# acoustic-warfare/beamforming-lk

Measured on AMD Instinct MI355X. Metric: heatmap frames/sec, higher is better.
Workload: dtype f32

## Files before the change

beamforming-lk_amd/_build.py:

```python
from __future__ import annotations

import os
import shutil
import subprocess
from pathlib import Path

PKG_DIR = Path(__file__).resolve().parent
REPO = PKG_DIR.parent
CSRC = PKG_DIR / "csrc"
LIB_PATH = PKG_DIR / "libawpu_hip.so"

SOURCES = [CSRC / "das_kernels.hip", CSRC / "das_fast.hip", CSRC / "track_kernels.hip", CSRC / "block_kernels.hip", CSRC / "watch_kernels.hip",
           CSRC / "awpu_hip.cpp", CSRC / "awpu_group.cpp", CSRC / "awpu_sweep.cpp", CSRC / "awpu_runs.cpp", CSRC / "geometry_host.cpp"]
GENERATOR = REPO / "tools" / "gen_trip_asm.py"
TRIP_INC = CSRC / "das_fast_trip.inc"
HEADERS = [CSRC / "awpu_handle.h", CSRC / "das_kernels.h", CSRC / "block_kernels.h", CSRC / "watch_kernels.h", GENERATOR, REPO / "include" / "awpu_hip.h", REPO / "include" / "awpu_hip_track.h",
           REPO / "include" / "awpu_hip_blocks.h", REPO / "include" / "awpu_hip_listen.h", REPO / "include" / "awpu_hip_watch.h"]


def hipcc_path() -> str:
    for cand in (os.environ.get("HIPCC"), shutil.which("hipcc"), "/opt/rocm/bin/hipcc"):
        if cand and Path(cand).exists():
            return cand
    raise RuntimeError("hipcc not found: libawpu_hip.so cannot be built (there is no CPU fallback)")


def stale() -> bool:
    if not LIB_PATH.exists():
        return True
    built = LIB_PATH.stat().st_mtime
    return any(p.stat().st_mtime > built for p in SOURCES + HEADERS)
# ... 62 lines not shown
```

beamforming-lk_amd/csrc/awpu_handle.h:

```cpp
#pragma once

#include "awpu_hip.h"
#include "awpu_hip_track.h"

#include <hip/hip_runtime.h>

#include <algorithm>
#include <string>
#include <utility>
#include <vector>

#include "das_kernels.h"

namespace awpu::host {

void note_error(const std::string &text);

struct CtxScope {
    awpu_hip *saved;
    explicit CtxScope(awpu_hip *h);
    ~CtxScope();
};
#define AWPU_CTX(h) awpu::host::CtxScope ctx_scope_(h)

// ... 195 lines not shown
    bool have_table = false, have_mics = false, prepared = false;

    Dev<awpu::LutEntry> d_lut;
    struct FastLut {
        awpu::FastPlan plan;
        Dev<awpu::FastEntry> d;
        size_t entries = 0;
    };
    std::vector<FastLut> fast_luts;
    Dev<awpu::FastEntry> d_exact_pair_lut;
    size_t exact_pair_lut_entries = 0, fir_plane_lut_entries = 0;
    awpu::FastPlan exact_plan{};
    awpu::host::QuadTable quad_tables[awpu::host::kQuadLayouts];
    Dev<unsigned> d_nd_queue;
    Dev<int2> d_nd_items;
    long long nd_items_key = -1;
    int n_cus = 0;
    bool exact_nd_ok = false;
    bool exact_ndh_ok = false, exact_ndhs_ok = false, fast_ndp_ok = false;
    bool identity_mics = false;
    bool exact_pairs_ok = false;
    float *sums_out = nullptr;
    Dev<uint32_t> d_fir_plane_lut;
    awpu::FastPlan fir_plane_plan{};
    bool fir_planes_ok = false;
    std::vector<float> fir;
    bool quadh_fits = false;
    bool quadhs_fits = false;
    bool quad_ok = false;
    double quad_cost = 0.0;
// ... 156 lines not shown
```

beamforming-lk_amd/csrc/awpu_sweep.cpp:

```cpp
#include "awpu_handle.h"

#include <algorithm>
#include <array>
#include <cstdio>
#include <cstdlib>
#include <cstring>
#include <map>
#include <vector>

#include "das_kernels.h"

using namespace awpu::host;

namespace {

int diag_begin(awpu_hip *h, size_t words, bool zero, hipStream_t s, unsigned long long **out) {
    if (const int rc = h->d_diag.ensure(words); rc != AWPU_OK) return rc;
    if (zero) AWPU_HIP_TRY(hipMemsetAsync(h->d_diag, 0, words * sizeof(unsigned long long), s));
    *out = h->d_diag;
    return AWPU_OK;
}

int diag_end(awpu_hip *h, int rc, size_t n_waves, int wg_waves, const char *tag, hipStream_t s) {
    if (rc != AWPU_OK || n_waves == 0) return rc;
    AWPU_HIP_TRY(hipStreamSynchronize(s));
// ... 76 lines not shown
    return AWPU_OK;
}
#endif

int ensure_pack(awpu_hip *h, size_t need) { return ensure_seen_by_live_graphs(h, h->d_pack, need); }

}

namespace awpu::host {

void free_tables(awpu_hip *h) {
    h->d_lut.release();
    h->fast_luts.clear();
    h->d_exact_pair_lut.release();
    for (QuadTable &q : h->quad_tables) q.d.release();
    h->d_fir_plane_lut.release();
}

int prepare(awpu_hip *h) {
    const auto &c = h->cfg;
    const int U = h->usable();
    const int P = c.pixel_count;
    int lo = c.hist, hi = -1;
    for (int p = 0; p < P; p++) {
        const int32_t *row = &h->off[(size_t) p * c.lut_stride];
        for (int s = 0; s < U; s++) {
            const int o = row[h->index[s]];
            lo = std::min(lo, o);
            hi = std::max(hi, o);
        }
// ... 41 lines not shown
                for (int q = 0; q < 2; q++) rr[2 * s + q] = h->index[s] * 2048 + lo + q;
            if (const int rc = h->d_row_off_ring.grow(rr.size()); rc != AWPU_OK) return rc;
            AWPU_HIP_TRY(hipMemcpy(h->d_row_off_ring, rr.data(), rr.size() * sizeof(int32_t), hipMemcpyHostToDevice));
        }
        if (h->compact_hist) {
            for (int s = 0; s < U; s++)
                for (int q = 0; q < 2; q++) ro[2 * s + q] = h->index[s] * h->compact_hist + q;
            for (size_t i = 2 * (size_t) U; i < ro.size(); i++) ro[i] = h->index[0] * h->compact_hist;
            if (const int rc = h->d_row_off_compact.grow(ro.size()); rc != AWPU_OK) return rc;
            AWPU_HIP_TRY(hipMemcpy(h->d_row_off_compact, ro.data(), ro.size() * sizeof(int32_t), hipMemcpyHostToDevice));
        }
    }

    h->exact_pairs_ok = c.math == AWPU_MATH_F32_EXACT && c.interp == AWPU_INTERP_LERP && awpu::pair_plan(h->window, U, &h->exact_plan);
    h->quad_tables[kQuadExact].plan = h->exact_plan;
    h->exact_nd_ok = h->exact_pairs_ok && awpu::exact_nd_plan(h->window, U, &h->quad_tables[kQuadExactNd].plan);
    h->exact_ndh_ok = h->exact_pairs_ok && awpu::exact_ndh_plan(h->window, U, false, &h->quad_tables[kQuadExactNdh].plan);
    h->fast_ndp_ok = c.math == AWPU_MATH_F32_FAST && c.interp == AWPU_INTERP_LERP && awpu::exact_ndh_plan(h->window, U, false, &h->quad_tables[kQuadExactNdh].plan);
    h->exact_ndhs_ok = h->exact_pairs_ok && awpu::exact_ndh_plan(h->window, U, true, &h->quad_tables[kQuadExactNdhStationary].plan);
    h->fir_planes_ok = c.math == AWPU_MATH_F32_FAST && c.interp == AWPU_INTERP_FIR8 && awpu::fir8_plane_plan(h->window, U, &h->fir_plane_plan);
    if (c.math != AWPU_MATH_F32_FAST || c.interp == AWPU_INTERP_FIR8) {
        int chunk = 0;
        if (awpu::das_exact_lds_bytes(h->window, U, &chunk) == 0)
            return invalid("delay window does not fit the LDS budget");
        std::vector<awpu::LutEntry> packed((size_t) P * U);
        for (int p = 0; p < P; p++) {
            const int32_t *orow = &h->off[(size_t) p * c.lut_stride];
            const float *frow = &h->frac[(size_t) p * c.lut_stride];
            awpu::LutEntry *dst = &packed[(size_t) p * U];
            for (int s = 0; s < U; s++) {
                const int id = h->index[s];
// ... 127 lines not shown
    }
    if (const int rc = lut.d.grow(n); rc != AWPU_OK) return rc;
    AWPU_HIP_TRY(hipMemcpy(lut.d, packed.data(), n * sizeof(awpu::FastEntry), hipMemcpyHostToDevice));
    lut.entries = n;
    h->fast_luts.reserve(8);
    h->fast_luts.push_back(std::move(lut));
    *out = &h->fast_luts.back();
    return AWPU_OK;
}

int build_quad_lut(awpu_hip *h, QuadLayout layout) {
    QuadTable &table = h->quad_tables[layout];
    if (table.d) return AWPU_OK;
    const auto &c = h->cfg;
    const awpu::FastPlan &plan = table.plan;
    const bool halves_nd = layout == kQuadExactNdh || layout == kQuadExactNdhStationary;
    const bool raw = layout == kQuadExact || layout == kQuadExactNd || halves_nd;
    const float centre = raw ? 0.0f : 0.5f;
    const int elem = layout == kQuadExactNd || halves_nd ? 16 : 8;
    const int U = h->usable(), cols = c.grid_columns, rows = c.pixel_count / cols;
    const int groups = plan.usable_pad / 4;
    const int cols_pad = halves_nd ? (cols + 31) / 32 * 32 : (cols + 15) / 16 * 16, rows4 = layout == kQuadExactNd ? ((rows + 3) / 4 + 1) / 2 * 2 : (rows + 3) / 4;
    const size_t n = (size_t) rows4 * cols_pad * groups * 16 + 2 * awpu::kQuadTablePrefetch;
    std::vector<awpu::QuadEntry> packed(n, awpu::QuadEntry{0.0f, 0u});
    for (int r4 = 0; r4 < rows4; r4++)
        for (int col = 0; col < cols_pad; col++) {
            awpu::QuadEntry *dst = &packed[((size_t) r4 * cols_pad + col) * groups * 16];
            for (int q = 0; q < 4; q++) {
                const int row = 4 * r4 + q;
                const bool inside = row < rows && col < cols;
                const size_t p = (size_t) std::min(row, rows - 1) * cols + std::min(col, cols - 1);
                const int32_t *orow = &h->off[p * c.lut_stride];
                const float *frow = &h->frac[p * c.lut_stride];
                for (int s = 0; s < plan.usable_pad; s++) {
                    awpu::QuadEntry &e = dst[((s >> 2) * 4 + q) * 4 + (s & 3)];
                    const int j = s % plan.chunk;
                    if (s < U) {
                        const int id = h->index[s];
                        const int off_rel = orow[id] - h->wstart;
                        e.f = inside ? frow[id] - centre : 0.0f;
                        e.addr = (uint32_t) (j * plan.row_bytes + off_rel * elem);
                    } else {
                        e.f = 0.0f;
                        e.addr = (uint32_t) (j * plan.row_bytes);
                    }
                }
            }
        }
    if (const int rc = table.d.grow(n); rc != AWPU_OK) return rc;
    AWPU_HIP_TRY(hipMemcpy(table.d, packed.data(), n * sizeof(awpu::QuadEntry), hipMemcpyHostToDevice));
    table.entries = n;
    return AWPU_OK;
}

// ... 165 lines not shown

int launch_exact_nd(awpu_hip *h, const float *d_frames, int batch, float *d_power, hipStream_t s, int hist_eff, int wstart_eff, int nq,
                    const float *prepacked = nullptr, size_t prepacked_floats = 0) {
    int rc = build_quad_lut(h, kQuadExactNd);
    if (rc != AWPU_OK) return rc;
    const QuadTable &table = h->quad_tables[kQuadExactNd];
    const awpu::FastPlan &pp = table.plan;
    if (!prepacked)
        if (const int prc = ensure_pack(h, pair_pack_floats(std::max(h->cfg.max_batch, batch), pp.usable_pad, pp.wr, 4)); prc != AWPU_OK) return prc;
    awpu::ExactNdArgs a{};
    fill_shared(a, h, pp, batch, d_power);
    a.packed = prepacked ? prepacked : h->d_pack;
    a.lut = table.d;
    a.sums = h->sums_out;
    a.wq = pp.wr;
    a.cols = h->cfg.grid_columns;
    a.rows = h->cfg.pixel_count / a.cols;
    a.nq = nq;
    a.tiles = awpu::nd_tiles(a.rows, a.cols, nq);
    a.n_pairs = (batch + 1) / 2;
    a.pair_group = xcd_pair_group((size_t) pp.usable_pad * pp.row_bytes, a.n_pairs);
    {
        const size_t items = (size_t) a.n_pairs * a.tiles;
        const long long key = ((long long) a.n_pairs << 24) | ((long long) a.pair_group << 8) | nq;
        if (!h->d_nd_items.holds(items)) {
            retire_live_graphs(h);
            AWPU_HIP_TRY(hipStreamSynchronize(s));
            if (rc = h->d_nd_items.grow(items); rc != AWPU_OK) return rc;
            h->nd_items_key = -1;
        }
        a.items = h->d_nd_items;
        a.build_items = h->nd_items_key != key;
        h->nd_items_key = key;
    }
    if (rc = arm_item_queues(h, a.n_pairs * a.tiles, &a.queue, &a.wgs, &a.tail); rc != AWPU_OK) return rc;
#ifdef AWPU_TUNING_BUILD
    if (const char *v = std::getenv("AWPU_ND_TAIL")) {
        const int per = (a.n_pairs * a.tiles + 7) / 8;
        a.tail = std::max(1, std::atoi(v) >= 100 ? per : per * std::atoi(v) / 100);
    }
#endif
    if (h->timing) AWPU_HIP_TRY(hipEventRecord(h->ev_begin, s));
    if (!prepacked)
        AWPU_HIP_TRY(awpu::launch_pack_nd(d_frames, h->cfg.n_streams, hist_eff, wstart_eff, h->d_index, h->usable(), pp.usable_pad, h->d_gain,
                                          pp.wr, batch, h->d_pack, s));
#ifdef AWPU_TUNING_BUILD
    const size_t n_wgs = std::min<size_t>((size_t) a.n_pairs * a.tiles, (size_t) a.wgs);
    if (env().debug & 16)
        if (const int drc = diag_begin(h, n_wgs * 8, true, s, &a.debug_out); drc != AWPU_OK) return drc;
#endif
    AWPU_HIP_TRY(awpu::launch_das_exact_nd(a, {table.entries, prepacked ? prepacked_floats : h->d_pack.cap}, s));
    rc = finish_launch(h, batch, s, AWPU_KERNEL_EXACT_ND);
#ifdef AWPU_TUNING_BUILD
    if (rc == AWPU_OK && (env().debug & 16)) return dump_nd_timeline(h, n_wgs, s);
#endif
    return rc;
}

bool takes_exact_nd(awpu_hip *h, int batch, int *nq) {
    if (!h->exact_pairs_ok || !h->exact_nd_ok || h->cfg.grid_columns < 1) return false;
// ... 425 lines not shown

bool takes_packed_pairs(awpu_hip *h, int batch, awpu::FastPlan *plan) {
    if (batch < 2 || h->cfg.interp != AWPU_INTERP_LERP || h->usable() % 4 != 0 || !h->gain.empty()) return false;
    if (h->cfg.math == AWPU_MATH_F32_EXACT) {
        int nq = 1;
        if (!takes_exact_nd(h, batch, &nq)) return false;
        *plan = h->quad_tables[kQuadExactNd].plan;
        return true;
    }
    if (h->cfg.math != AWPU_MATH_F32_FAST || env().pairs == 0) return false;
    if (!awpu::pair_plan(h->window, h->usable(), plan)) return false;
    return (fast_batch_takes_quads(h, batch) && quad_plan_is(h, *plan)) || fast_batch_takes_pairs(h, batch);
}

size_t packed_floats_of(const awpu_hip *h, const awpu::FastPlan &plan, int batch) {
    return (size_t) ((batch + 1) / 2) * h->usable() * (size_t) (plan.row_bytes / 4);
}

int pack_for_sweep(awpu_hip *h, const awpu::FastPlan &plan, const float *d_frames, int batch, float *d_packed, hipStream_t s) {
    if (h->cfg.math == AWPU_MATH_F32_EXACT)
        AWPU_HIP_TRY(awpu::launch_pack_nd(d_frames, h->cfg.n_streams, h->cfg.hist, h->wstart, h->d_index, h->usable(), h->usable(), nullptr, plan.wr,
                                          batch, d_packed, s));
    else
        AWPU_HIP_TRY(awpu::launch_pack_pairs(d_frames, h->cfg.n_streams, h->cfg.hist, h->wstart, h->d_index, h->usable(), h->usable(), nullptr,
                                             plan.wr, batch, d_packed, true, s));
    return AWPU_OK;
}

int sweep_packed(awpu_hip *h, const awpu::FastPlan &plan, const float *d_packed, size_t packed_floats, int batch, float *d_power,
                 hipStream_t s) {
    if (h->cfg.math == AWPU_MATH_F32_EXACT) {
        int nq = 1;
        if (!takes_exact_nd(h, batch, &nq)) return fail(AWPU_ERR_STATE, "packed frames: this batch is not swept by the {next, d} kernel");
        return launch_exact_nd(h, nullptr, batch, d_power, s, h->cfg.hist, h->wstart, nq, d_packed, packed_floats);
    }
    if (fast_batch_takes_quads(h, batch) && quad_plan_is(h, plan))
        return launch_quads(h, nullptr, batch, d_power, s, h->cfg.hist, h->wstart, d_packed, packed_floats);
// ... 24 lines not shown
```

beamforming-lk_amd/csrc/das_fast.hip:

```cpp
#include "das_kernels.h"

#include <algorithm>
#include <atomic>

namespace awpu {

typedef float f2 __attribute__((ext_vector_type(2)));
typedef float f4 __attribute__((ext_vector_type(4)));
typedef float f4u __attribute__((ext_vector_type(4), aligned(4)));
typedef float f8 __attribute__((ext_vector_type(8)));

#define AWPU_AS4 __attribute__((address_space(4)))

typedef int i16 __attribute__((ext_vector_type(16)));

struct EntryGroup {
    i16 v;
    __device__ __forceinline__ float f(int k) const { return __int_as_float(v[4 * k + 0]); }
    __device__ __forceinline__ unsigned addr(int k) const { return (unsigned) v[4 * k + 1]; }
    __device__ __forceinline__ float g(int k) const { return __int_as_float(v[4 * k + 2]); }
};

template <int FPI>
struct Reads {
// ... 1076 lines not shown
    {
        const float total = wave_sum8(s0.x, s0.y, s1.x, s1.y, s2.x, s2.y, s3.x, s3.y, lane);
        const int value = kWaveSum8Value(lane >> 3), row = 4 * row4 + (value >> 1), frame = 2 * pair + (value & 1);
        if ((lane & 7) == 0 && row < a.rows && col < a.cols && frame < a.batch)
            a.power[(size_t) frame * a.pixel_count + (size_t) row * a.cols + col] = total / norm;
    }
}

__device__ __forceinline__ f2 next_and_difference(float cur, float next, float gm) {
#pragma clang fp contract(off)
    const float c = cur * gm, n = next * gm;
    return f2{n, c - n};
}

__global__ void pack_nd_kernel(const float *frames, int n_streams, int hist, int wstart, const int32_t *index, int usable,
                               const float *gain, int wq, int batch, float *packed) {
    const int pair = blockIdx.y, s = blockIdx.x, rows_out = gridDim.x;
    f4 *dst = (f4 *) packed + ((size_t) pair * rows_out + s) * wq;
    if (s >= usable) {
        for (int t = threadIdx.x; t < wq; t += blockDim.x) dst[t] = f4{0.0f, 0.0f, 0.0f, 0.0f};
        return;
    }
    const int fa = min(2 * pair, batch - 1), fb = min(2 * pair + 1, batch - 1);
    const float *xa = frames + ((size_t) fa * n_streams + index[s]) * hist + wstart;
    const float *xb = frames + ((size_t) fb * n_streams + index[s]) * hist + wstart;
    const float gm = gain ? gain[s] : 1.0f;
    const int valid = min(wq, hist - wstart - 1);
    for (int t = threadIdx.x; t < wq; t += blockDim.x) {
        f4 v = f4{0.0f, 0.0f, 0.0f, 0.0f};
        if (t < valid) {
            const f2 ea = next_and_difference(xa[t], xa[t + 1], gm), eb = next_and_difference(xb[t], xb[t + 1], gm);
            v = f4{ea.x, eb.x, ea.y, eb.y};
// ... 33 lines not shown
            if (run >= 8) return -1;
            if (k < len(run) - head(run)) return run * per + head(run) + k;
        }
    }
    __device__ __forceinline__ int take(int xcd) const {
        int item = take_head(xcd);
        if (item < 0) item = take_common();
        for (int y = 1; item < 0 && y < 8; y++) item = take_head((xcd + y) & 7);
        return item;
    }
};

template <int NQ, bool SUMS>
__global__ __launch_bounds__(1024, 4) void das_exact_nd_kernel(ExactNdArgs a) {
    extern __shared__ __attribute__((aligned(16))) float lds[];
    constexpr int NW = 16, kThreads = NW * 64, BUF = kFastLdsBytes;
    constexpr int kPieces = (BUF + kThreads * 16 - 1) / (kThreads * 16);
    const int wave = __builtin_amdgcn_readfirstlane(threadIdx.x >> 6);
    const unsigned lds_base = (unsigned) (unsigned long long) (const __attribute__((address_space(3))) char *) lds;
    int *mail = (int *) (lds + 2 * (BUF / 4));
    const int total = a.n_pairs * a.tiles;
    unsigned xcc;
    asm volatile("s_getreg_b32 %0, hwreg(HW_REG_XCC_ID)" : "=s"(xcc));
    const NdQueues Q{a.queue, (total + 7) >> 3, total, a.tail};
    const int xcd = (int) (xcc & 7u);
    if (threadIdx.x == 0) {
        const int first = Q.take(xcd);
        mail[0] = first;
        mail[1] = first >= 0 ? Q.take(xcd) : -1;
    }
    __syncthreads();
    int cur = __builtin_amdgcn_readfirstlane(mail[0]), nxt = __builtin_amdgcn_readfirstlane(mail[1]);
    if (cur < 0) return;
    __syncthreads();

    auto decode = [&](int item, int &pair, int &tile_quad) {
        const int2 d = a.items[item];
        pair = __builtin_amdgcn_readfirstlane(d.x);
        tile_quad = __builtin_amdgcn_readfirstlane(d.y);
    };
    const int tiles_per_row = (a.cols + NW - 1) / NW;
    const int groups_total = a.usable_pad >> 2;
    const size_t row_floats = (size_t) a.wq * 4;
    const int n_chunks = (a.usable_pad + a.chunk - 1) / a.chunk;
    const int first_mics = min(a.chunk, a.usable_pad), last_mics = a.usable_pad - (n_chunks - 1) * a.chunk;
    const int ngf = __builtin_amdgcn_readfirstlane(first_mics >> 2), ngl = __builtin_amdgcn_readfirstlane(last_mics >> 2);
    const unsigned dbf = __builtin_amdgcn_readfirstlane((unsigned) ((size_t) a.chunk * row_floats * 4));
    const unsigned dbl = __builtin_amdgcn_readfirstlane((unsigned) ((size_t) last_mics * row_floats * 4));
    const unsigned db0 = __builtin_amdgcn_readfirstlane((unsigned) ((size_t) first_mics * row_floats * 4));
    const int rank = wave >> 2;
    const int own_head = Q.head(xcd);

    int pair, tile;
    decode(cur, pair, tile);
#ifdef AWPU_TUNING_BUILD
    const unsigned long long rt_begin = a.debug_out ? __builtin_amdgcn_s_memrealtime() : 0ull;
    long long t_sweep = 0, t_other = 0, t_mark = __builtin_readcyclecounter();
    int n_items = 0;
#endif
    {
        const float *pair_base = a.packed + (size_t) pair * a.usable_pad * row_floats;
        const int n_pieces = (int) ((size_t) first_mics * row_floats / 4);
#pragma unroll
        for (int k = 0; k < kPieces; k++) {
            const int piece = threadIdx.x + k * kThreads;
            if (piece < n_pieces) {
                float *dst = lds + (wave * 64 + k * kThreads) * 4;
                __builtin_amdgcn_global_load_lds((const __attribute__((address_space(1))) void *) (pair_base + (size_t) piece * 4),
                                                 (__attribute__((address_space(3))) void *) dst, 16, 0, 0);
            }
        }
    }
    asm volatile("s_waitcnt vmcnt(0)" ::: "memory");
    __syncthreads();
    unsigned step = 0;

    for (;;) {
        const int cols_pad = tiles_per_row * NW;
        const int rowq = tile / (NQ * cols_pad);
        const int col = tile - NQ * rowq * cols_pad + wave;
        const int quad0 = tile + wave;
        const QuadEntry *quad_lut = a.lut + (size_t) quad0 * groups_total * 16;
        const float *pair_base = a.packed + (size_t) pair * a.usable_pad * row_floats;
        int pair_next = pair, tile_next = tile;
        if (nxt >= 0) decode(nxt, pair_next, tile_next);
        const float *next_base = a.packed + (size_t) pair_next * a.usable_pad * row_floats;
        unsigned ticket = 0;
        const bool asked = wave == 0 && nxt >= 0 && own_head > 0;
        const unsigned *qptr = (const unsigned *) uniform_ptr(asked ? a.queue + xcd : nullptr);

        f8 O[NQ][4];
#ifdef AWPU_TUNING_BUILD
        { const long long n = __builtin_readcyclecounter(); t_other += n - t_mark; t_mark = n; }
#endif
        {
            unsigned tid = threadIdx.x;
            asm volatile("" : "+v"(tid));
            const unsigned lane_bytes = tid * 16;
            const int buf = (int) (step & 1);
            unsigned lane_addr = lds_base + buf * BUF + (tid & 63) * 16;
            const unsigned ddst = __builtin_amdgcn_readfirstlane(lds_base + (buf ^ 1) * BUF + wave * 1024);
            const int delta = __builtin_amdgcn_readfirstlane(buf ? -BUF : BUF);
            const unsigned dbn = __builtin_amdgcn_readfirstlane(nxt >= 0 ? db0 : 0u);
            if constexpr (NQ == 1) {
                sweep_exact_nd_item1(O[0][0], O[0][1], O[0][2], O[0][3], uniform_ptr(quad_lut), ngf, ngl, __builtin_amdgcn_readfirstlane(n_chunks),
                                     lane_addr, rank, uniform_ptr(pair_base), dbf, dbl, uniform_ptr(next_base), dbn, ddst, delta, lane_bytes, qptr, ticket);
            } else {
                static_assert(NQ == 2, "blocks are generated for one and two quads per wave");
                const int qstride = __builtin_amdgcn_readfirstlane(tiles_per_row * NW * groups_total * 16 * (int) sizeof(QuadEntry));
                sweep_exact_nd_item2(O[0][0], O[0][1], O[0][2], O[0][3], O[1][0], O[1][1], O[1][2], O[1][3], uniform_ptr(quad_lut), qstride, ngf, ngl,
                                     __builtin_amdgcn_readfirstlane(n_chunks), lane_addr, rank, uniform_ptr(pair_base), dbf, dbl, uniform_ptr(next_base),
                                     dbn, ddst, delta, lane_bytes, qptr, ticket);
            }
            step += n_chunks;
        }
        if (threadIdx.x == 0 && nxt >= 0) {
            int got = own_head > 0 && ticket < (unsigned) own_head ? xcd * Q.per + (int) ticket : -1;
            if (got < 0) {
                got = Q.take_common();
                for (int y = 1; got < 0 && y < 8; y++) got = Q.take_head((xcd + y) & 7);
            }
            mail[0] = got;
        }
#ifdef AWPU_TUNING_BUILD
        { const long long n = __builtin_readcyclecounter(); t_sweep += n - t_mark; t_mark = n; n_items++; }
#endif

// ... 20 lines not shown
                }
                return pixel_pair_partial_exact(o, lane);
            };
            const f2 s0 = finish(O[q][0], 0), s1 = finish(O[q][1], 1), s2 = finish(O[q][2], 2), s3 = finish(O[q][3], 3);
            const float sum = wave_sum8(s0.x, s0.y, s1.x, s1.y, s2.x, s2.y, s3.x, s3.y, lane);
            const int value = kWaveSum8Value(lane >> 3), row = 4 * row4 + (value >> 1), frame = 2 * pair + (value & 1);
            if ((lane & 7) == 0 && row < a.rows && col < a.cols && frame < a.batch)
                a.power[(size_t) frame * a.pixel_count + (size_t) row * a.cols + col] = sum / norm;
        }

        if (nxt < 0) break;
        __syncthreads();
        cur = nxt;
        pair = pair_next;
        tile = tile_next;
        nxt = __builtin_amdgcn_readfirstlane(mail[0]);
        __syncthreads();
    }
#ifdef AWPU_TUNING_BUILD
    if (a.debug_out && threadIdx.x == 0) {
        unsigned hw_id;
        asm volatile("s_getreg_b32 %0, hwreg(HW_REG_HW_ID)" : "=s"(hw_id));
        unsigned long long *o = a.debug_out + 8 * (size_t) blockIdx.x;
        o[0] = rt_begin;
        o[1] = __builtin_amdgcn_s_memrealtime();
        o[2] = (unsigned long long) t_other;
        o[3] = (unsigned long long) t_sweep;
        o[4] = (unsigned long long) (__builtin_readcyclecounter() - t_mark);
        o[5] = ((unsigned long long) xcc << 32) | hw_id;
        o[6] = (unsigned long long) n_items;
// ... 1058 lines not shown
                       (const FirPlaneEntry *) d_entries, d_coeffs, n_tiles, g);
    return hipGetLastError();
}

hipError_t launch_das_fir8_planes(const PairArgs &a, const void *d_entries, const float *d_coeffs, int variant, const Extents &have,
                                  hipStream_t stream) {
#ifdef AWPU_QUAD_VARIANTS
    if (variant == 1) return launch_fir8_plane_variant<1>(a, d_entries, d_coeffs, have, stream);
    if (variant == 2) return launch_fir8_plane_variant<2>(a, d_entries, d_coeffs, have, stream);
    if (variant == 3) return launch_fir8_plane_variant<3>(a, d_entries, d_coeffs, have, stream);
#endif
    (void) variant;
    return launch_fir8_plane_variant<0>(a, d_entries, d_coeffs, have, stream);
}

bool exact_nd_plan(int window, int usable, FastPlan *plan) {
    const int wq = window - 1;
    const size_t row_bytes = (size_t) wq * 16;
    int chunk = (int) ((size_t) kFastLdsBytes / row_bytes);
    chunk &= ~3;
    if (chunk > 64) chunk = 64;
    if (chunk < 4 || wq < kSamples) return false;
    const int usable_pad = (usable + 3) & ~3;
    if (chunk > usable_pad) chunk = usable_pad;
    plan->fpi = 2;
    plan->wr = wq;
    plan->chunk = chunk;
    plan->usable_pad = usable_pad;
    plan->row_bytes = (int) row_bytes;
    plan->image_bytes = -4;
    return true;
}

hipError_t launch_pack_nd(const float *d_frames, int n_streams, int hist, int wstart, const int32_t *d_index, int usable, int rows_out,
                          const float *d_gain, int wq, int batch, float *d_packed, hipStream_t stream) {
    hipLaunchKernelGGL(pack_nd_kernel, dim3(rows_out, (batch + 1) / 2), dim3(128), 0, stream, d_frames, n_streams, hist, wstart, d_index,
                       usable, d_gain, wq, batch, d_packed);
    return hipGetLastError();
}

template <int NQ, bool SUMS>
static hipError_t launch_exact_nd_variant(const ExactNdArgs &a, hipStream_t stream) {
    static LdsFlags attr_set = {};
    constexpr int lds_bytes = 2 * kFastLdsBytes + 64;
    if (hipError_t e = allow_lds((const void *) das_exact_nd_kernel<NQ, SUMS>, lds_bytes, attr_set); e != hipSuccess) return e;
    const long total = (long) a.n_pairs * a.tiles;
    if (hipError_t e = hipMemsetAsync(a.queue, 0, 9 * sizeof(unsigned), stream); e != hipSuccess) return e;
    if (a.build_items)
        hipLaunchKernelGGL(nd_items_kernel, dim3((unsigned) ((total + 255) / 256)), dim3(256), 0, stream, const_cast<int2 *>(a.items), a.n_pairs,
                           a.tiles, a.pair_group, (a.cols + 15) / 16, NQ);
    hipLaunchKernelGGL((das_exact_nd_kernel<NQ, SUMS>), dim3((unsigned) std::min<long>(total, std::max(1, a.wgs))), dim3(1024), lds_bytes, stream, a);
    return hipGetLastError();
}

hipError_t launch_das_exact_nd(const ExactNdArgs &a, const Extents &have, hipStream_t stream) {
    if ((a.nq != 1 && a.nq != 2) || !a.queue || !a.items || a.wgs < 1 || a.tail < 1) return hipErrorInvalidValue;
    if (a.chunk < 4 || (a.chunk & 3) || (a.usable_pad & 3) || a.usable < 1 || a.usable > a.usable_pad || a.wq < kSamples ||
        (size_t) a.chunk * a.wq * 16 > (size_t) kFastLdsBytes || a.cols < 1 || a.rows * a.cols != a.pixel_count)
        return hipErrorInvalidValue;
    if (a.n_pairs != (a.batch + 1) / 2 || a.tiles != nd_tiles(a.rows, a.cols, a.nq) || a.pair_group < 1) return hipErrorInvalidValue;
    if (!within({(size_t) nd_quad_count(a.rows, a.cols, a.nq) * (a.usable_pad / 4) * 16 + kQuadTablePrefetch,
                 (size_t) a.n_pairs * a.usable_pad * a.wq * 4}, have))
        return hipErrorInvalidValue;
    if (a.sums) return a.nq == 2 ? launch_exact_nd_variant<2, true>(a, stream) : launch_exact_nd_variant<1, true>(a, stream);
    return a.nq == 2 ? launch_exact_nd_variant<2, false>(a, stream) : launch_exact_nd_variant<1, false>(a, stream);
}

bool exact_ndh_plan(int window, int usable, bool stationary, FastPlan *plan) {
    const int wh = window - 129;
    if (wh < kSamples / 2) return false;
    const size_t row_bytes = (size_t) wh * 16;
    const int usable_pad = (usable + 3) & ~3;
    int chunk;
    if (stationary) {
        if ((size_t) usable_pad * row_bytes > (size_t) 2 * kFastLdsBytes) return false;
// ... 258 lines not shown
```

beamforming-lk_amd/csrc/das_kernels.h:

```cpp
#pragma once

#include <hip/hip_runtime.h>
#include <stdint.h>

namespace awpu {

constexpr int kSamples = 256;

constexpr int kDebugNoRefill = 1, kDebugNoSweep = 2, kDebugNoTail = 4, kDebugNoBarrier = 8, kDebugRegStaging = 64;
constexpr int kDebugSafeBits = 16 | 256 | 512 | 4096;
#if defined(AWPU_TIMING_BUILD) && !defined(AWPU_TUNING_BUILD)
#define AWPU_TUNING_BUILD 1
#endif
#ifdef AWPU_TIMING_BUILD
#define AWPU_DBG(a, bit) ((a).debug & (bit))
#else
#define AWPU_DBG(a, bit) 0
#endif

struct LutEntry {
    int32_t off_rel;
    float frac;
};

// ... 86 lines not shown
};
hipError_t launch_das_exact_pairs(const ExactPairArgs &a, const Extents &have, hipStream_t stream);
struct ExactQuadArgs {
    const float *packed;
    const struct QuadEntry *lut;
    float *power;
    float *sums;
    int32_t usable, usable_pad, pixel_count, wp, chunk, batch;
    int32_t cols, rows;
    int32_t tiles, n_pairs, pair_group;
};
hipError_t launch_das_exact_quads(const ExactQuadArgs &a, const Extents &have, hipStream_t stream);
struct ExactNdArgs {
    const float *packed;
    const struct QuadEntry *lut;
    float *power;
    float *sums;
    int32_t usable, usable_pad, pixel_count, wq, chunk, batch;
    int32_t cols, rows;
    int32_t nq;
    int32_t tiles, n_pairs, pair_group;
    unsigned *queue;
    int32_t wgs;
    int32_t tail;
    const int2 *items;
    int32_t build_items;
    unsigned long long *debug_out;
};
inline int nd_tiles(int rows, int cols, int nq) { return (((rows + 3) / 4 + nq - 1) / nq) * ((cols + 15) / 16); }
inline int nd_quad_count(int rows, int cols, int nq) { return (((rows + 3) / 4 + nq - 1) / nq) * nq * ((cols + 15) / 16) * 16; }
bool exact_nd_plan(int window, int usable, FastPlan *plan);
hipError_t launch_pack_nd(const float *d_frames, int n_streams, int hist, int wstart, const int32_t *d_index, int usable, int rows_out,
                          const float *d_gain, int wq, int batch, float *d_packed, hipStream_t stream);
hipError_t launch_das_exact_nd(const ExactNdArgs &a, const Extents &have, hipStream_t stream);
struct DoneFlag {
    unsigned long long *counter;
    unsigned *flag;
    unsigned long long target;
    uint32_t seq;
};
struct ExactNdhArgs {
    const float *packed;
    const float *frames;
    const struct QuadEntry *lut;
    const int32_t *index;
    const float *gain;
    float *power;
    float *sums;
// ... 208 lines not shown
```

Measured before the change: 23230.

## Load per-tile delay windows into LDS for the exact ND sweep

On the host, computes for each 8x16 pixel tile and each mic the minimum delay offset and the overall spread, then narrows the per-mic row staged in LDS to 256+spread samples starting at a per-tile offset. The LUT addresses are rebased against these starts, and the kernel loads one row per wave from a per-tile start table. This cuts LDS traffic and global loads per item, and lets more mics fit in each chunk. The change also moves zeroing of the work queue into the pack kernel so one memset is dropped, and lets pair grouping rise to 4 when the working set is small. The risks are that the sweep assembly blocks take a new packed argument signature, and that the chunk size is now capped at 16 mics.

```diff
diff --git a/beamforming-lk_amd/_build.py b/beamforming-lk_amd/_build.py
--- a/beamforming-lk_amd/_build.py
+++ b/beamforming-lk_amd/_build.py
@@ -14,7 +14,7 @@
            CSRC / "awpu_hip.cpp", CSRC / "awpu_group.cpp", CSRC / "awpu_sweep.cpp", CSRC / "awpu_runs.cpp", CSRC / "geometry_host.cpp"]
 GENERATOR = REPO / "tools" / "gen_trip_asm.py"
 TRIP_INC = CSRC / "das_fast_trip.inc"
-HEADERS = [CSRC / "awpu_handle.h", CSRC / "das_kernels.h", CSRC / "block_kernels.h", CSRC / "watch_kernels.h", GENERATOR, REPO / "include" / "awpu_hip.h", REPO / "include" / "awpu_hip_track.h",
+HEADERS = [CSRC / "awpu_handle.h", CSRC / "das_kernels.h", CSRC / "block_kernels.h", CSRC / "watch_kernels.h", CSRC / "nd_tile_window.h", GENERATOR, REPO / "include" / "awpu_hip.h", REPO / "include" / "awpu_hip_track.h",
            REPO / "include" / "awpu_hip_blocks.h", REPO / "include" / "awpu_hip_listen.h", REPO / "include" / "awpu_hip_watch.h"]
 
 
diff --git a/beamforming-lk_amd/csrc/awpu_handle.h b/beamforming-lk_amd/csrc/awpu_handle.h
--- a/beamforming-lk_amd/csrc/awpu_handle.h
+++ b/beamforming-lk_amd/csrc/awpu_handle.h
@@ -233,6 +233,8 @@
     awpu::host::QuadTable quad_tables[awpu::host::kQuadLayouts];
     Dev<unsigned> d_nd_queue;
     Dev<int2> d_nd_items;
+    Dev<unsigned> d_nd_starts;
+    size_t nd_start_entries = 0;
     long long nd_items_key = -1;
     int n_cus = 0;
     bool exact_nd_ok = false;
diff --git a/beamforming-lk_amd/csrc/awpu_sweep.cpp b/beamforming-lk_amd/csrc/awpu_sweep.cpp
--- a/beamforming-lk_amd/csrc/awpu_sweep.cpp
+++ b/beamforming-lk_amd/csrc/awpu_sweep.cpp
@@ -9,6 +9,7 @@
 #include <vector>
 
 #include "das_kernels.h"
+#include "nd_tile_window.h"
 
 using namespace awpu::host;
 
@@ -115,6 +116,7 @@
     h->fast_luts.clear();
     h->d_exact_pair_lut.release();
     for (QuadTable &q : h->quad_tables) q.d.release();
+    h->d_nd_starts.release();
     h->d_fir_plane_lut.release();
 }
 
@@ -186,7 +188,7 @@
 
     h->exact_pairs_ok = c.math == AWPU_MATH_F32_EXACT && c.interp == AWPU_INTERP_LERP && awpu::pair_plan(h->window, U, &h->exact_plan);
     h->quad_tables[kQuadExact].plan = h->exact_plan;
-    h->exact_nd_ok = h->exact_pairs_ok && awpu::exact_nd_plan(h->window, U, &h->quad_tables[kQuadExactNd].plan);
+    h->exact_nd_ok = h->exact_pairs_ok && awpu::exact_nd_plan(h->window, U, 0, &h->quad_tables[kQuadExactNd].plan);
     h->exact_ndh_ok = h->exact_pairs_ok && awpu::exact_ndh_plan(h->window, U, false, &h->quad_tables[kQuadExactNdh].plan);
     h->fast_ndp_ok = c.math == AWPU_MATH_F32_FAST && c.interp == AWPU_INTERP_LERP && awpu::exact_ndh_plan(h->window, U, false, &h->quad_tables[kQuadExactNdh].plan);
     h->exact_ndhs_ok = h->exact_pairs_ok && awpu::exact_ndh_plan(h->window, U, true, &h->quad_tables[kQuadExactNdhStationary].plan);
@@ -344,6 +346,18 @@
     if (table.d) return AWPU_OK;
     const auto &c = h->cfg;
     const awpu::FastPlan &plan = table.plan;
+    std::vector<uint16_t> starts;
+    if (layout == kQuadExactNd) {
+        const int cols = c.grid_columns, wq = plan.wr;
+        const int wq_tile = awpu::nd_tile_windows(h->off.data(), c.lut_stride, h->index.data(), h->usable(), plan.usable_pad, c.pixel_count / cols, cols,
+                                                  h->wstart, wq, &starts);
+        if (!awpu::exact_nd_plan(h->window, h->usable(), wq_tile, &table.plan)) return fail(AWPU_ERR_STATE, "the {next, d} image does not hold the tile window");
+        std::vector<unsigned> bytes(starts.size() + 16, 0u);
+        for (size_t i = 0; i < starts.size(); i++) bytes[i] = 16u * starts[i];
+        if (const int rc = h->d_nd_starts.grow(bytes.size()); rc != AWPU_OK) return rc;
+        AWPU_HIP_TRY(hipMemcpy(h->d_nd_starts, bytes.data(), bytes.size() * sizeof(unsigned), hipMemcpyHostToDevice));
+        h->nd_start_entries = bytes.size();
+    }
     const bool halves_nd = layout == kQuadExactNdh || layout == kQuadExactNdhStationary;
     const bool raw = layout == kQuadExact || layout == kQuadExactNd || halves_nd;
     const float centre = raw ? 0.0f : 0.5f;
@@ -367,7 +381,9 @@
                     const int j = s % plan.chunk;
                     if (s < U) {
                         const int id = h->index[s];
-                        const int off_rel = orow[id] - h->wstart;
+                        int off_rel = orow[id] - h->wstart;
+                        if (layout == kQuadExactNd)
+                            off_rel -= starts[((size_t) (r4 / 2) * (cols_pad / 16) + col / 16) * plan.usable_pad + s];
                         e.f = inside ? frow[id] - centre : 0.0f;
                         e.addr = (uint32_t) (j * plan.row_bytes + off_rel * elem);
                     } else {
@@ -563,12 +579,16 @@
     a.lut = table.d;
     a.sums = h->sums_out;
     a.wq = pp.wr;
+    a.wq_tile = pp.row_bytes / 16;
+    a.starts = h->d_nd_starts;
+    a.start_entries = h->nd_start_entries;
     a.cols = h->cfg.grid_columns;
     a.rows = h->cfg.pixel_count / a.cols;
     a.nq = nq;
     a.tiles = awpu::nd_tiles(a.rows, a.cols, nq);
     a.n_pairs = (batch + 1) / 2;
-    a.pair_group = xcd_pair_group((size_t) pp.usable_pad * pp.row_bytes, a.n_pairs);
+    a.pair_group = xcd_pair_group((size_t) pp.usable_pad * pp.wr * 16, a.n_pairs, env().pair_group);
+    if (env().pair_group <= 0 && a.pair_group == 2 && a.n_pairs >= 4 && (size_t) pp.usable_pad * pp.wr * 16 * 4 <= (6u << 20)) a.pair_group = 4;
     {
         const size_t items = (size_t) a.n_pairs * a.tiles;
         const long long key = ((long long) a.n_pairs << 24) | ((long long) a.pair_group << 8) | nq;
@@ -590,9 +610,11 @@
     }
 #endif
     if (h->timing) AWPU_HIP_TRY(hipEventRecord(h->ev_begin, s));
-    if (!prepacked)
+    if (!prepacked) {
         AWPU_HIP_TRY(awpu::launch_pack_nd(d_frames, h->cfg.n_streams, hist_eff, wstart_eff, h->d_index, h->usable(), pp.usable_pad, h->d_gain,
-                                          pp.wr, batch, h->d_pack, s));
+                                          pp.wr, batch, h->d_pack, a.queue, s));
+        a.queue_zeroed = 1;
+    }
 #ifdef AWPU_TUNING_BUILD
     const size_t n_wgs = std::min<size_t>((size_t) a.n_pairs * a.tiles, (size_t) a.wgs);
     if (env().debug & 16)
@@ -1048,13 +1070,13 @@
 }
 
 size_t packed_floats_of(const awpu_hip *h, const awpu::FastPlan &plan, int batch) {
-    return (size_t) ((batch + 1) / 2) * h->usable() * (size_t) (plan.row_bytes / 4);
+    return (size_t) ((batch + 1) / 2) * h->usable() * (size_t) (plan.image_bytes == -4 ? plan.wr * 4 : plan.row_bytes / 4);
 }
 
 int pack_for_sweep(awpu_hip *h, const awpu::FastPlan &plan, const float *d_frames, int batch, float *d_packed, hipStream_t s) {
     if (h->cfg.math == AWPU_MATH_F32_EXACT)
         AWPU_HIP_TRY(awpu::launch_pack_nd(d_frames, h->cfg.n_streams, h->cfg.hist, h->wstart, h->d_index, h->usable(), h->usable(), nullptr, plan.wr,
-                                          batch, d_packed, s));
+                                          batch, d_packed, nullptr, s));
     else
         AWPU_HIP_TRY(awpu::launch_pack_pairs(d_frames, h->cfg.n_streams, h->cfg.hist, h->wstart, h->d_index, h->usable(), h->usable(), nullptr,
                                              plan.wr, batch, d_packed, true, s));
diff --git a/beamforming-lk_amd/csrc/das_fast.hip b/beamforming-lk_amd/csrc/das_fast.hip
--- a/beamforming-lk_amd/csrc/das_fast.hip
+++ b/beamforming-lk_amd/csrc/das_fast.hip
@@ -1,4 +1,5 @@
 #include "das_kernels.h"
+#include "nd_tile_window.h"
 
 #include <algorithm>
 #include <atomic>
@@ -1114,8 +1115,9 @@
 }
 
 __global__ void pack_nd_kernel(const float *frames, int n_streams, int hist, int wstart, const int32_t *index, int usable,
-                               const float *gain, int wq, int batch, float *packed) {
+                               const float *gain, int wq, int batch, float *packed, unsigned *queue) {
     const int pair = blockIdx.y, s = blockIdx.x, rows_out = gridDim.x;
+    if (queue && pair == 0 && s == 0 && threadIdx.x < 9) queue[threadIdx.x] = 0u;
     f4 *dst = (f4 *) packed + ((size_t) pair * rows_out + s) * wq;
     if (s >= usable) {
         for (int t = threadIdx.x; t < wq; t += blockDim.x) dst[t] = f4{0.0f, 0.0f, 0.0f, 0.0f};
@@ -1179,8 +1181,7 @@
 template <int NQ, bool SUMS>
 __global__ __launch_bounds__(1024, 4) void das_exact_nd_kernel(ExactNdArgs a) {
     extern __shared__ __attribute__((aligned(16))) float lds[];
-    constexpr int NW = 16, kThreads = NW * 64, BUF = kFastLdsBytes;
-    constexpr int kPieces = (BUF + kThreads * 16 - 1) / (kThreads * 16);
+    constexpr int NW = 16, BUF = kFastLdsBytes;
     const int wave = __builtin_amdgcn_readfirstlane(threadIdx.x >> 6);
     const unsigned lds_base = (unsigned) (unsigned long long) (const __attribute__((address_space(3))) char *) lds;
     int *mail = (int *) (lds + 2 * (BUF / 4));
@@ -1199,40 +1200,49 @@
     if (cur < 0) return;
     __syncthreads();
 
-    auto decode = [&](int item, int &pair, int &tile_quad) {
+    const int tiles_per_row = (a.cols + NW - 1) / NW;
+    auto decode = [&](int item, int &pair, int &tile_quad, const unsigned *&starts) {
         const int2 d = a.items[item];
         pair = __builtin_amdgcn_readfirstlane(d.x);
         tile_quad = __builtin_amdgcn_readfirstlane(d.y);
+        const int quad_row = (tile_quad >> 4) / tiles_per_row, col_tile = (tile_quad >> 4) - quad_row * tiles_per_row;
+        starts = a.starts + (size_t) ((quad_row >> 1) * tiles_per_row + col_tile) * a.usable_pad;
     };
-    const int tiles_per_row = (a.cols + NW - 1) / NW;
     const int groups_total = a.usable_pad >> 2;
     const size_t row_floats = (size_t) a.wq * 4;
     const int n_chunks = (a.usable_pad + a.chunk - 1) / a.chunk;
     const int first_mics = min(a.chunk, a.usable_pad), last_mics = a.usable_pad - (n_chunks - 1) * a.chunk;
-    const int ngf = __builtin_amdgcn_readfirstlane(first_mics >> 2), ngl = __builtin_amdgcn_readfirstlane(last_mics >> 2);
     const unsigned dbf = __builtin_amdgcn_readfirstlane((unsigned) ((size_t) a.chunk * row_floats * 4));
-    const unsigned dbl = __builtin_amdgcn_readfirstlane((unsigned) ((size_t) last_mics * row_floats * 4));
-    const unsigned db0 = __builtin_amdgcn_readfirstlane((unsigned) ((size_t) first_mics * row_floats * 4));
+    const int row_bytes = a.wq_tile * 16;
+    const int row_pieces = (row_bytes + 1023) >> 10;
+    const unsigned last_shift = (unsigned) (row_pieces * 64 - a.wq_tile);
     const int rank = wave >> 2;
+    const unsigned pka = __builtin_amdgcn_readfirstlane((unsigned) (first_mics >> 2) | (unsigned) (last_mics >> 2) << 8 | (unsigned) n_chunks << 16);
+    const unsigned pkb_item = (wave < a.chunk ? (unsigned) row_pieces : 0u) | (wave < last_mics ? (unsigned) row_pieces : 0u) << 8 | last_shift << 24 |
+                              (unsigned) rank << 30;
+    const unsigned pkb_next = wave < first_mics ? (unsigned) row_pieces << 16 : 0u;
     const int own_head = Q.head(xcd);
 
     int pair, tile;
-    decode(cur, pair, tile);
+    const unsigned *starts;
+    decode(cur, pair, tile, starts);
 #ifdef AWPU_TUNING_BUILD
     const unsigned long long rt_begin = a.debug_out ? __builtin_amdgcn_s_memrealtime() : 0ull;
     long long t_sweep = 0, t_other = 0, t_mark = __builtin_readcyclecounter();
     int n_items = 0;
 #endif
     {
-        const float *pair_base = a.packed + (size_t) pair * a.usable_pad * row_floats;
-        const int n_pieces = (int) ((size_t) first_mics * row_floats / 4);
-#pragma unroll
-        for (int k = 0; k < kPieces; k++) {
-            const int piece = threadIdx.x + k * kThreads;
-            if (piece < n_pieces) {
-                float *dst = lds + (wave * 64 + k * kThreads) * 4;
-                __builtin_amdgcn_global_load_lds((const __attribute__((address_space(1))) void *) (pair_base + (size_t) piece * 4),
-                                                 (__attribute__((address_space(3))) void *) dst, 16, 0, 0);
+        if (wave < first_mics) {
+            const unsigned start = __builtin_amdgcn_readfirstlane(starts[wave]);
+            const float *src = a.packed + ((size_t) pair * a.usable_pad + wave) * row_floats + (start >> 2);
+            const int lane = (int) (threadIdx.x & 63);
+            for (int k = 0; k < row_pieces; k++) {
+                const int el = k * 64 + lane;
+                if (el < a.wq_tile) {
+                    float *dst = lds + ((wave * row_bytes) >> 2) + k * 256;
+                    __builtin_amdgcn_global_load_lds((const __attribute__((address_space(1))) void *) (src + (size_t) el * 4),
+                                                     (__attribute__((address_space(3))) void *) dst, 16, 0, 0);
+                }
             }
         }
     }
@@ -1248,7 +1258,8 @@
         const QuadEntry *quad_lut = a.lut + (size_t) quad0 * groups_total * 16;
         const float *pair_base = a.packed + (size_t) pair * a.usable_pad * row_floats;
         int pair_next = pair, tile_next = tile;
-        if (nxt >= 0) decode(nxt, pair_next, tile_next);
+        const unsigned *starts_next = starts;
+        if (nxt >= 0) decode(nxt, pair_next, tile_next, starts_next);
         const float *next_base = a.packed + (size_t) pair_next * a.usable_pad * row_floats;
         unsigned ticket = 0;
         const bool asked = wave == 0 && nxt >= 0 && own_head > 0;
@@ -1261,21 +1272,22 @@
         {
             unsigned tid = threadIdx.x;
             asm volatile("" : "+v"(tid));
-            const unsigned lane_bytes = tid * 16;
+            const unsigned lane_bytes = (tid & 63) * 16;
             const int buf = (int) (step & 1);
-            unsigned lane_addr = lds_base + buf * BUF + (tid & 63) * 16;
-            const unsigned ddst = __builtin_amdgcn_readfirstlane(lds_base + (buf ^ 1) * BUF + wave * 1024);
+            unsigned lane_addr = lds_base + buf * BUF + lane_bytes;
+            const unsigned ddst = __builtin_amdgcn_readfirstlane(lds_base + (buf ^ 1) * BUF + wave * row_bytes);
             const int delta = __builtin_amdgcn_readfirstlane(buf ? -BUF : BUF);
-            const unsigned dbn = __builtin_amdgcn_readfirstlane(nxt >= 0 ? db0 : 0u);
+            const unsigned pkb = __builtin_amdgcn_readfirstlane(pkb_item | (nxt >= 0 ? pkb_next : 0u));
+            const float *row_src = pair_base + (size_t) wave * row_floats, *row_next = next_base + (size_t) wave * row_floats;
             if constexpr (NQ == 1) {
-                sweep_exact_nd_item1(O[0][0], O[0][1], O[0][2], O[0][3], uniform_ptr(quad_lut), ngf, ngl, __builtin_amdgcn_readfirstlane(n_chunks),
-                                     lane_addr, rank, uniform_ptr(pair_base), dbf, dbl, uniform_ptr(next_base), dbn, ddst, delta, lane_bytes, qptr, ticket);
+                sweep_exact_nd_item1(O[0][0], O[0][1], O[0][2], O[0][3], uniform_ptr(quad_lut), pka, lane_addr, pkb, uniform_ptr(row_src), dbf,
+                                     uniform_ptr(row_next), ddst, delta, lane_bytes, uniform_ptr(starts + wave), uniform_ptr(starts_next + wave), qptr, ticket);
             } else {
                 static_assert(NQ == 2, "blocks are generated for one and two quads per wave");
                 const int qstride = __builtin_amdgcn_readfirstlane(tiles_per_row * NW * groups_total * 16 * (int) sizeof(QuadEntry));
-                sweep_exact_nd_item2(O[0][0], O[0][1], O[0][2], O[0][3], O[1][0], O[1][1], O[1][2], O[1][3], uniform_ptr(quad_lut), qstride, ngf, ngl,
-                                     __builtin_amdgcn_readfirstlane(n_chunks), lane_addr, rank, uniform_ptr(pair_base), dbf, dbl, uniform_ptr(next_base),
-                                     dbn, ddst, delta, lane_bytes, qptr, ticket);
+                sweep_exact_nd_item2(O[0][0], O[0][1], O[0][2], O[0][3], O[1][0], O[1][1], O[1][2], O[1][3], uniform_ptr(quad_lut), qstride, pka, lane_addr,
+                                     pkb, uniform_ptr(row_src), dbf, uniform_ptr(row_next), ddst, delta, lane_bytes, uniform_ptr(starts + wave),
+                                     uniform_ptr(starts_next + wave), qptr, ticket);
             }
             step += n_chunks;
         }
@@ -1326,6 +1338,7 @@
         cur = nxt;
         pair = pair_next;
         tile = tile_next;
+        starts = starts_next;
         nxt = __builtin_amdgcn_readfirstlane(mail[0]);
         __syncthreads();
     }
@@ -2414,13 +2427,13 @@
     return launch_fir8_plane_variant<0>(a, d_entries, d_coeffs, have, stream);
 }
 
-bool exact_nd_plan(int window, int usable, FastPlan *plan) {
+bool exact_nd_plan(int window, int usable, int wq_tile, FastPlan *plan) {
     const int wq = window - 1;
-    const size_t row_bytes = (size_t) wq * 16;
-    int chunk = (int) ((size_t) kFastLdsBytes / row_bytes);
-    chunk &= ~3;
-    if (chunk > 64) chunk = 64;
-    if (chunk < 4 || wq < kSamples) return false;
+    if (wq_tile <= 0 || wq_tile > wq) wq_tile = wq;
+    const size_t row_bytes = (size_t) wq_tile * 16;
+    if (wq_tile < kSamples) return false;
+    int chunk = nd_chunk_mics(wq_tile, kFastLdsBytes);
+    if (chunk < 4) return false;
     const int usable_pad = (usable + 3) & ~3;
     if (chunk > usable_pad) chunk = usable_pad;
     plan->fpi = 2;
@@ -2433,9 +2446,9 @@
 }
 
 hipError_t launch_pack_nd(const float *d_frames, int n_streams, int hist, int wstart, const int32_t *d_index, int usable, int rows_out,
-                          const float *d_gain, int wq, int batch, float *d_packed, hipStream_t stream) {
+                          const float *d_gain, int wq, int batch, float *d_packed, unsigned *d_queue, hipStream_t stream) {
     hipLaunchKernelGGL(pack_nd_kernel, dim3(rows_out, (batch + 1) / 2), dim3(128), 0, stream, d_frames, n_streams, hist, wstart, d_index,
-                       usable, d_gain, wq, batch, d_packed);
+                       usable, d_gain, wq, batch, d_packed, d_queue);
     return hipGetLastError();
 }
 
@@ -2445,7 +2458,8 @@
     constexpr int lds_bytes = 2 * kFastLdsBytes + 64;
     if (hipError_t e = allow_lds((const void *) das_exact_nd_kernel<NQ, SUMS>, lds_bytes, attr_set); e != hipSuccess) return e;
     const long total = (long) a.n_pairs * a.tiles;
-    if (hipError_t e = hipMemsetAsync(a.queue, 0, 9 * sizeof(unsigned), stream); e != hipSuccess) return e;
+    if (!a.queue_zeroed)
+        if (hipError_t e = hipMemsetAsync(a.queue, 0, 9 * sizeof(unsigned), stream); e != hipSuccess) return e;
     if (a.build_items)
         hipLaunchKernelGGL(nd_items_kernel, dim3((unsigned) ((total + 255) / 256)), dim3(256), 0, stream, const_cast<int2 *>(a.items), a.n_pairs,
                            a.tiles, a.pair_group, (a.cols + 15) / 16, NQ);
@@ -2455,10 +2469,11 @@
 
 hipError_t launch_das_exact_nd(const ExactNdArgs &a, const Extents &have, hipStream_t stream) {
     if ((a.nq != 1 && a.nq != 2) || !a.queue || !a.items || a.wgs < 1 || a.tail < 1) return hipErrorInvalidValue;
-    if (a.chunk < 4 || (a.chunk & 3) || (a.usable_pad & 3) || a.usable < 1 || a.usable > a.usable_pad || a.wq < kSamples ||
-        (size_t) a.chunk * a.wq * 16 > (size_t) kFastLdsBytes || a.cols < 1 || a.rows * a.cols != a.pixel_count)
+    if (a.chunk < 4 || (a.chunk & 3) || a.chunk > 16 || (a.usable_pad & 3) || a.usable < 1 || a.usable > a.usable_pad || a.wq_tile < kSamples ||
+        a.wq_tile > a.wq || (size_t) a.chunk * a.wq_tile * 16 > (size_t) kFastLdsBytes || a.cols < 1 || a.rows * a.cols != a.pixel_count)
         return hipErrorInvalidValue;
     if (a.n_pairs != (a.batch + 1) / 2 || a.tiles != nd_tiles(a.rows, a.cols, a.nq) || a.pair_group < 1) return hipErrorInvalidValue;
+    if (!a.starts || a.start_entries < (size_t) nd_tiles(a.rows, a.cols, 2) * a.usable_pad + 16) return hipErrorInvalidValue;
     if (!within({(size_t) nd_quad_count(a.rows, a.cols, a.nq) * (a.usable_pad / 4) * 16 + kQuadTablePrefetch,
                  (size_t) a.n_pairs * a.usable_pad * a.wq * 4}, have))
         return hipErrorInvalidValue;
diff --git a/beamforming-lk_amd/csrc/das_kernels.h b/beamforming-lk_amd/csrc/das_kernels.h
--- a/beamforming-lk_amd/csrc/das_kernels.h
+++ b/beamforming-lk_amd/csrc/das_kernels.h
@@ -124,6 +124,9 @@
 struct ExactNdArgs {
     const float *packed;
     const struct QuadEntry *lut;
+    const unsigned *starts;
+    size_t start_entries;
+    int32_t wq_tile;
     float *power;
     float *sums;
     int32_t usable, usable_pad, pixel_count, wq, chunk, batch;
@@ -131,6 +134,7 @@
     int32_t nq;
     int32_t tiles, n_pairs, pair_group;
     unsigned *queue;
+    int32_t queue_zeroed;
     int32_t wgs;
     int32_t tail;
     const int2 *items;
@@ -139,9 +143,9 @@
 };
 inline int nd_tiles(int rows, int cols, int nq) { return (((rows + 3) / 4 + nq - 1) / nq) * ((cols + 15) / 16); }
 inline int nd_quad_count(int rows, int cols, int nq) { return (((rows + 3) / 4 + nq - 1) / nq) * nq * ((cols + 15) / 16) * 16; }
-bool exact_nd_plan(int window, int usable, FastPlan *plan);
+bool exact_nd_plan(int window, int usable, int wq_tile, FastPlan *plan);
 hipError_t launch_pack_nd(const float *d_frames, int n_streams, int hist, int wstart, const int32_t *d_index, int usable, int rows_out,
-                          const float *d_gain, int wq, int batch, float *d_packed, hipStream_t stream);
+                          const float *d_gain, int wq, int batch, float *d_packed, unsigned *d_queue, hipStream_t stream);
 hipError_t launch_das_exact_nd(const ExactNdArgs &a, const Extents &have, hipStream_t stream);
 struct DoneFlag {
     unsigned long long *counter;
diff --git a/beamforming-lk_amd/csrc/nd_tile_window.h b/beamforming-lk_amd/csrc/nd_tile_window.h
--- /dev/null
+++ b/beamforming-lk_amd/csrc/nd_tile_window.h
@@ -0,0 +1,40 @@
+#pragma once
+#include <algorithm>
+#include <cstddef>
+#include <cstdint>
+#include <vector>
+
+namespace awpu {
+
+inline int nd_chunk_mics(int wq_tile, int image_bytes) { return std::min(16, (int) ((size_t) image_bytes / ((size_t) wq_tile * 16)) & ~3); }
+
+inline int nd_window_tiles(int rows, int cols) { return (((rows + 3) / 4 + 1) / 2) * ((cols + 15) / 16); }
+
+inline int nd_tile_windows(const int32_t *off, int lut_stride, const int32_t *index, int usable, int usable_pad, int rows, int cols, int wstart, int wq,
+                           std::vector<uint16_t> *start) {
+    const int tiles_per_row = (cols + 15) / 16, tiles = nd_window_tiles(rows, cols);
+    std::vector<int32_t> lo((size_t) tiles * usable_pad, 0);
+    int spread = 0;
+    for (int t = 0; t < tiles; t++) {
+        const int r0 = 8 * (t / tiles_per_row), c0 = 16 * (t % tiles_per_row);
+        for (int s = 0; s < usable; s++) {
+            int mn = INT32_MAX, mx = INT32_MIN;
+            for (int r = r0; r < r0 + 8; r++)
+                for (int c = c0; c < c0 + 16; c++) {
+                    const size_t p = (size_t) std::min(r, rows - 1) * cols + std::min(c, cols - 1);
+                    const int v = off[p * lut_stride + index[s]] - wstart;
+                    mn = std::min(mn, v);
+                    mx = std::max(mx, v);
+                }
+            lo[(size_t) t * usable_pad + s] = mn;
+            spread = std::max(spread, mx - mn);
+        }
+    }
+    const int wq_tile = std::min(wq, 256 + spread);
+    start->assign((size_t) tiles * usable_pad, 0);
+    if (wq_tile < wq && wq - wq_tile <= 0xffff)
+        for (size_t i = 0; i < lo.size(); i++) (*start)[i] = (uint16_t) std::min(lo[i], wq - wq_tile);
+    return wq_tile < wq && wq - wq_tile <= 0xffff ? wq_tile : wq;
+}
+
+}
```

After: 23580, median of 6. +1.5%, better.
